# fuine/katome

Hardware: AMD Instinct MI355X
Metric: k-mers/s (higher is better)
Workload: dtype u64

## Files before the change

### katome_amd/csrc/lds_count.hip

```cpp
#include <algorithm>

#include "common.h"
#include "lds_order.h"
#include "lds_plan.h"
#include "slot_bits.h"

namespace katome {

#ifdef KATOME_LC_PHASES
__device__ unsigned long long lc_phase_cycles[16];
#define LC_PHASE_BEGIN() unsigned long long lc_t0 = clock64()
#define LC_PHASE(i) do { if (threadIdx.x == 0) { const unsigned long long lc_t = clock64(); atomicAdd(&lc_phase_cycles[i], lc_t - lc_t0); lc_t0 = lc_t; } } while (0)
#else
#define LC_PHASE_BEGIN() do {} while (0)
#define LC_PHASE(i) do {} while (0)
#endif
template <int PER> KD u32 lc_step(u64 h) {
#ifdef KATOME_LC_LINEAR
    return 1u;
#else
    u32 step = (u32)((h >> 33) & 0x1FFu) * 2u + 1u;
    if ((PER & (PER - 1)) != 0 && step % (u32)PER == 0) step += 2;
    return step;
#endif
}

template <int NW, int STRIDE = NW>
__global__ __launch_bounds__(BLOCK) void hash_group_index_kernel(const u64* __restrict__ keys, u64 n, u32 gbits, u64* __restrict__ index) {
    for (u64 g = (u64)blockIdx.x * BLOCK + threadIdx.x; g <= (1ull << gbits); g += (u64)gridDim.x * BLOCK) {
        u64 lo = 0, hi = n;
        while (lo < hi) {
            const u64 mid = lo + ((hi - lo) >> 1);
            Key<NW> a;
#pragma unroll
            for (int q = 0; q < NW; ++q) a.w[q] = keys[mid * STRIDE + q];
            if ((hash_key(a) >> (64 - gbits)) < g) lo = mid + 1; else hi = mid;
        }
        index[g] = lo;
    }
}

template <bool RC, int PER, bool EVEN_K>
__global__ __launch_bounds__(LC_THREADS) void lds_count_kernel(const u64* keys, const u32* wts, const u64* __restrict__ index, u32 gbits,
                                                                u32 R, u32 k, u32 min_weight, u64* out_keys,
                                                                u32* out_w, u64 out_cap, unsigned long long* cursor,
                                                                unsigned long long* distinct, u32* err, u32 probe_limit,
                                                                unsigned long long* owner_cursor, u32 n_owners) {
    constexpr u32 LC_SLOTS = LcTable<PER>::SLOTS;
    extern __shared__ unsigned long long lc_mem[];
    unsigned long long* lkey = lc_mem;
    u32* lcnt = reinterpret_cast<u32*>(lc_mem + LC_SLOTS);
    __shared__ u32 wtot[LC_THREADS / 64];
    __shared__ unsigned long long base_sh;
    const u32 tid = threadIdx.x, lane = tid & 63, wave = tid >> 6;
    u32 my_distinct = 0;
    LC_PHASE_BEGIN();
    const u32 n_groups = 1u << gbits, sub_shift = 64 - gbits - 16;
    for (u32 g = blockIdx.x; g < n_groups; g += gridDim.x) {
        const u64 lo = index[g], hi = index[g + 1];
        if (lo == hi) continue;
        for (u32 r = 0; r < R; ++r) {
            for (u32 i = tid; i < LC_SLOTS; i += LC_THREADS) { lkey[i] = 0ull; lcnt[i] = 0u; }
            __syncthreads();
            LC_PHASE(0);
            constexpr u32 LU = KATOME_LC_LU;
            for (u64 i0 = lo + tid; i0 < hi; i0 += (u64)LC_THREADS * LU) {
                u64 kv[LU]; u32 wv[LU];
#pragma unroll
// ... 147 lines not shown
                const unsigned long long v = slot[tid * LP_PER + j];
                kk[j].w[0] = 0; cc[j] = 0;
                if (v) {
                    ++my_distinct;
                    cc[j] = (u32)v & 0xFFFFu;
                    kk[j].w[0] = unmix64(((u64)g << 48) | (v >> 16));
                    if (cc[j] >= min_weight) keep |= 1u << j;
                }
            }
            const u32 mine = (u32)__popc(keep);
            u32 incl = mine;
#pragma unroll
            for (int o = 1; o < 64; o <<= 1) { u32 t = __shfl_up(incl, o, 64); if (lane >= (u32)o) incl += t; }
            if (lane == 63) wtot[wave] = incl;
            __syncthreads();
            u32 woff = 0, total = 0;
#pragma unroll
            for (u32 w = 0; w < LC_THREADS / 64; ++w) { if (w < wave) woff += wtot[w]; total += wtot[w]; }
            constexpr u32 F = RC ? 2 : 1;
            if (tid == 0) base_sh = total ? atomicAdd(cursor, (unsigned long long)total * F) : 0ull;
            __syncthreads();
            LC_PHASE(10);
            {
                unsigned long long* skey = lc_mem;
                u32* sw = reinterpret_cast<u32*>(lc_mem + LP_STAGE);
                const u32 p0 = woff + (incl - mine);
                for (u32 c0 = 0; c0 < total; c0 += LP_STAGE) {
                    u32 p = p0 - c0;
#pragma unroll
                    for (u32 j = 0; j < LP_PER; ++j) {
                        if (!((keep >> j) & 1u)) continue;
                        if (p < LP_STAGE) { skey[p] = kk[j].w[0]; sw[p] = cc[j]; }
                        ++p;
                    }
                    __syncthreads();
                    const u32 nc = total - c0 < LP_STAGE ? total - c0 : LP_STAGE;
                    const u64 o0 = base_sh + (u64)c0 * F;
                    for (u32 o = tid; o < nc * F; o += LC_THREADS) {
                        const u32 e = RC ? o >> 1 : o;
                        Key<1> x; x.w[0] = skey[e];
                        if (RC && (o & 1u)) x = revcomp(x, k);
                        if (o0 + o < out_cap) { out_keys[o0 + o] = x.w[0]; out_w[o0 + o] = sw[e]; }
                    }
                    __syncthreads();
                }
            }
            LC_PHASE(11);
        }
    }
    my_distinct = wave_sum(my_distinct);
    if (lane == 0 && my_distinct) atomicAdd(distinct, (unsigned long long)my_distinct);
}

constexpr u32 LO_BUCKETS = LDS_ORDER_BUCKETS;
static_assert(LC_THREADS == LDS_ORDER_THREADS, "the read-out orders with lds_order.h");
template <bool RC>
__global__ __launch_bounds__(LC_THREADS) void lds_count_ordered_kernel(const u64* keys, const u32* wts, const u64* __restrict__ index, u32 k,
                                                                        u32 min_weight, u64* s1_key, u32* s1_w, u32* group_count, u64* s2_key,
                                                                        u32* s2_w, uint8_t* s2_digit, u64 s2_cap, unsigned long long* cursor,
                                                                        unsigned long long* distinct, u32* err, u32 probe_limit) {
    extern __shared__ unsigned long long lc_mem[];
    unsigned long long* slot = lc_mem;
    u32* bucket = reinterpret_cast<u32*>(lc_mem + LP_SLOTS);
    __shared__ u32 wtot[LC_THREADS / 64];
    __shared__ unsigned long long base_sh;
    const u32 tid = threadIdx.x, lane = tid & 63;
    const u32 rem_bits = 2 * k - 16, bshift = rem_bits > 11 ? rem_bits - 11 : 0;
    const u64 REM = (1ull << rem_bits) - 1;
    u32 my_distinct = 0;
    LC_PHASE_BEGIN();
    for (u32 g = blockIdx.x; g < (1u << 16); g += gridDim.x) {
        const u64 lo = index[g], hi = index[g + 1];
        if (lo == hi) continue;
        for (u32 i = tid; i < LP_SLOTS; i += LC_THREADS) slot[i] = 0ull;
        bucket[tid] = 0u;
        __syncthreads();
        LC_PHASE(12);
        constexpr u32 LU = KATOME_LC_LU;
        constexpr u32 NB = LP_SLOTS / 2;
        for (u64 i0 = lo + tid; i0 < hi; i0 += (u64)LC_THREADS * LU) {
            u64 kv[LU]; u32 wv[LU];
#pragma unroll
            for (u32 u = 0; u < LU; ++u) { const u64 i = i0 + (u64)u * LC_THREADS; kv[u] = 0; wv[u] = 0; if (i < hi) { kv[u] = keys[i]; wv[u] = wts[i]; } }
#pragma unroll
            for (u32 u = 0; u < LU; ++u) {
                const u64 i = i0 + (u64)u * LC_THREADS;
                if (i >= hi) continue;
                const u64 h = mix64(kv[u]);
                const u32 w = wv[u];
                if (w == 0u || w > 0xFFFFu) { *err = 5; continue; }
                const unsigned long long rem = kv[u] & REM, mine = (rem << 16) | w;
                u32 b0 = (u32)(((h & 0x3FFFFFFFull) * NB) >> 30);
                const u32 step = lc_step<LP_PER>(h);
                u32 probes = 0;
                for (; probes < probe_limit; ++probes) {
                    u32 b1 = b0 + step; if (b1 >= NB) b1 -= NB;
                    const ulonglong2 x = *reinterpret_cast<const ulonglong2*>(slot + 2 * b0), y = *reinterpret_cast<const ulonglong2*>(slot + 2 * b1);
                    const unsigned long long c[4] = {x.x, x.y, y.x, y.y};
                    u32 at = ~0u; bool have = false;
#pragma unroll
                    for (int j = 3; j >= 0; --j) if ((c[j] >> 16) == rem && c[j] != 0ull) { at = (j < 2 ? 2 * b0 : 2 * b1 - 2) + j; have = true; }
                    if (!have) {
#pragma unroll
                        for (int j = 3; j >= 0; --j) if (c[j] == 0ull) at = (j < 2 ? 2 * b0 : 2 * b1 - 2) + j;
                        if (at == ~0u) { b0 = b1 + step; if (b0 >= NB) b0 -= NB; continue; }
                        const unsigned long long cur = atomicCAS(&slot[at], 0ull, mine);
                        if (cur == 0ull) break;
                        if ((cur >> 16) != rem) continue;
                    }
                    const unsigned long long old = atomicAdd(&slot[at], (unsigned long long)w);
                    if ((old & 0xFFFFull) + w > 0xFFFFull) *err = 5;
                    break;
                }
                if (probes == probe_limit) *err = 3;
            }
        }
        __syncthreads();
        LC_PHASE(13);
        unsigned long long v[LP_PER]; u32 keep = 0;
#pragma unroll
        for (u32 j = 0; j < LP_PER; ++j) {
            v[j] = slot[tid * LP_PER + j];
            if (v[j]) { ++my_distinct; if (((u32)v[j] & 0xFFFFu) >= min_weight) keep |= 1u << j; }
        }
        const u32 total = lds_order_entries<LP_PER>(v, keep, slot, bucket, wtot, bshift, [&](u32 t) {
            if (tid == 0) { group_count[g] = t; base_sh = t ? atomicAdd(cursor, (unsigned long long)t) : 0ull; }
        });
        LC_PHASE(14);
        for (u32 i = tid; i < total; i += LC_THREADS) {
            const unsigned long long e = slot[i];
            Key<1> x; x.w[0] = ((u64)g << rem_bits) | (e >> 16);
            const u32 c = (u32)e & 0xFFFFu;
            if (lo + i < hi) { s1_key[lo + i] = x.w[0]; s1_w[lo + i] = c; }
            if (RC && base_sh + i < s2_cap) {
                const u64 r = revcomp(x, k).w[0];
                s2_key[base_sh + i] = r; s2_w[base_sh + i] = c; s2_digit[base_sh + i] = (uint8_t)(r >> rem_bits);
            }
        }
        __syncthreads();
        LC_PHASE(15);
    }
    my_distinct = wave_sum(my_distinct);
    if (lane == 0 && my_distinct) atomicAdd(distinct, (unsigned long long)my_distinct);
}

template <bool REP>
__global__ __launch_bounds__(BLOCK) void orient_records_kernel(u64* keys, u64 n, u32 k) {
    for (u64 i = (u64)blockIdx.x * BLOCK + threadIdx.x; i < n; i += (u64)gridDim.x * BLOCK) {
        Key<1> x; x.w[0] = keys[i];
        keys[i] = (REP ? rep_orientation(x, k) : canonical(x, k)).w[0];
    }
}

__global__ __launch_bounds__(BLOCK) void core_group_index_kernel(const u64* __restrict__ keys, u64 n, u32 gbits, u32 core_shift, u32 core_bases,
                                                                 u64* __restrict__ index) {
    for (u64 g = (u64)blockIdx.x * BLOCK + threadIdx.x; g <= (1ull << gbits); g += (u64)gridDim.x * BLOCK) {
        u64 lo = 0, hi = n;
        while (lo < hi) {
            const u64 mid = lo + ((hi - lo) >> 1);
            Key<1> a; a.w[0] = keys[mid];
            if ((core_hash(a, core_shift, core_bases) >> (64 - gbits)) < g) lo = mid + 1; else hi = mid;
        }
        index[g] = lo;
    }
}
__global__ void owner_bases_kernel(const u64* __restrict__ index, u32 gbits, u32 n_owners, unsigned long long* owner_cursor, u64* bases) {
    const u32 p = threadIdx.x;
    if (p > n_owners) return;
    const u64 g0 = (((u64)p << gbits) + n_owners - 1) / n_owners;
    const u64 at = index[g0 < (1ull << gbits) ? g0 : (1ull << gbits)];
    bases[p] = at;
    if (p < n_owners) owner_cursor[p] = at;
}

template <bool RC, int PER, int NW, bool EVEN_K>
__global__ __launch_bounds__(LC_THREADS) void lds_count_wide_kernel(const u64* keys, const u32* wts, const u64* __restrict__ index, u32 gbits,
                                                                     u32 R, u32 k, u32 min_weight, u64* out_keys, u32* out_w, u64 out_cap,
                                                                     unsigned long long* cursor, unsigned long long* distinct, u32* err, u32 probe_limit,
                                                                     unsigned long long* , u32 ) {
    constexpr u32 LC_SLOTS = LcTable<PER>::SLOTS;
    constexpr unsigned long long REP_MASK = (1ull << 20) - 1;
    extern __shared__ unsigned long long lc_mem[];
// ... 605 lines not shown
    const uint64_t out_cap = ((rc && !list) ? 2 : 1) * n + 2;
    KCHECK(edge_key.alloc(out_cap * 8 * (list ? stride : nwk), stream));
    KCHECK(seq_weight.alloc(out_cap * (list ? 4 : 16), stream));
    LcResult r;
    auto count = [&](u32 rounds, u32 probe_limit) -> int {
        auto launch = [&](auto kernel) {
            return lc_launch(aux, kernel, (size_t)LcsTable::SLOTS * 28, n, r, ko, wo, index.as<u64>(), gbits, rounds, k, seq_per_read, edge_key.as<u64>(),
                             seq_weight.as<u64>(), out_cap, aux.cursor(), aux.distinct(), aux.err(), probe_limit);
        };
        return with_bool(rc, [&](auto rcv) { return with_bool(list, [&](auto lv) {
            constexpr bool RC = decltype(rcv)::value, LIST = decltype(lv)::value;
            return nwk == 1 ? launch(lds_count_seen_kernel<RC, 1, LIST>) : launch(lds_count_seen_kernel<RC, 2, LIST>);
        }); });
    };
    KCHECK(count_optimistic("first-seen order", lc_rounds_try(avg, lc_optimism(), LcsTable::FILL), R, LcsTable::SLOTS, r, count));
    if (r.code == 4 || r.code == 6) return KATOME_E_UNSUPPORTED;
    if (r.code) { set_error("counting in LDS (first-seen order): a sub-round did not fit its table (code %u)", (unsigned)r.code); return KATOME_E_DEVICE; }
    *n_edges = r.n_out; *n_distinct = r.n_distinct;
    return KATOME_OK;
}

int table_orient_records(uint64_t* d_keys, uint64_t n, uint32_t k, bool rep, hipStream_t stream) {
    if (!n) return KATOME_OK;
    KernelScope ks(K_RECORDS, stream, n);
    if (rep) hipLaunchKernelGGL(orient_records_kernel<true>, dim3(grid_for(n, BLOCK, 256u * 32u)), dim3(BLOCK), 0, stream, d_keys, n, k);
    else     hipLaunchKernelGGL(orient_records_kernel<false>, dim3(grid_for(n, BLOCK, 256u * 32u)), dim3(BLOCK), 0, stream, d_keys, n, k);
    KCHECK_HIP(hipGetLastError());
    return KATOME_OK;
}

static int ordered_count(DevBuf& keys, DevBuf& weights, uint64_t n, uint32_t k, bool rc, uint32_t min_weight, HalfSort& hs, uint64_t* n_edges,
                         uint64_t* n_distinct, hipStream_t stream, uint32_t* first_counts) {
    if (!n || !weights.p || k < 9 || 2 * k > 62 || (rc && !(k & 1)) || !lp_group_fits(n >> 16)) return KATOME_E_UNSUPPORTED;
    const u64* ko = nullptr; const u32* wo = nullptr;
    {
        DevBuf kb(stream), wb(stream);
        KCHECK(kb.alloc((n + 1) * 8)); KCHECK(wb.alloc((n + 1) * 4));
        KCHECK(dev_key_order(keys.as<u64>(), weights.as<u32>(), n, k, kb.as<u64>(), keys.as<u64>(), wb.as<u32>(), weights.as<u32>(), &ko, &wo, stream, first_counts));
    }
    KCHECK(hs.group_first.alloc(((1ull << 16) + 1) * 8, stream));
    KCHECK(dev_key_group_index(ko, n, 2 * k - 16, hs.group_first.as<u64>(), stream));
    KCHECK(hs.group_count.alloc((1ull << 16) * 4, stream));
    KCHECK_HIP(hipMemsetAsync(hs.group_count.p, 0, (1ull << 16) * 4, stream));
    KCHECK(hs.s1_key.alloc((n + 1) * 8, stream)); KCHECK(hs.s1_w.alloc((n + 1) * 4, stream));
    const u64 s2_cap = rc ? n + 1 : 0;
    if (rc) {
        KCHECK(hs.s2_key.alloc(s2_cap * 8, stream)); KCHECK(hs.s2_w.alloc(s2_cap * 4, stream));
        KCHECK(hs.s2_digit.alloc(dev_digit_stream_bytes(s2_cap, 1), stream));
    }
    LcAux aux(stream);
    KCHECK(aux.buf.alloc(64));
    LcResult r;
    KCHECK(with_bool(rc, [&](auto rcv) {
        return lc_launch(aux, lds_count_ordered_kernel<decltype(rcv)::value>, (size_t)LP_SLOTS * 8 + LO_BUCKETS * 2, n, r, ko, wo, hs.group_first.as<u64>(), k,
                         min_weight, hs.s1_key.as<u64>(), hs.s1_w.as<u32>(), hs.group_count.as<u32>(), hs.s2_key.as<u64>(), hs.s2_w.as<u32>(),
                         hs.s2_digit.as<uint8_t>(), s2_cap, aux.cursor(), aux.distinct(), aux.err(), std::min<u32>(lc_probe_limit(), LP_SLOTS));
    }));
    lc_trace("[lds count] in key order, 8-byte slots, 1 visit(s) per record: code %u\n", (unsigned)r.code);
    if (r.code) {
        lc_trace("[lds count] in key order: %s; counting by hash groups\n", r.code == 5 ? "a count over 16 bits" : "a group filled its table");
        hs.release();
        return KATOME_E_UNSUPPORTED;
    }
    hs.n_s1 = r.n_out; hs.n_s2 = rc ? r.n_out : 0; hs.k = k; hs.taken = true;
    *n_edges = hs.n_s1 + hs.n_s2; *n_distinct = r.n_distinct;
    return KATOME_OK;
}

static bool s2_group_sort_on() { static const bool on = env_flag("KATOME_S2_GROUP_SORT", true); return on; }
static uint64_t s2_group_cap() {
    static const uint64_t cap = [] {
        const char* e = getenv("KATOME_S2_GROUP_CAP");
        const uint64_t c = e ? strtoull(e, nullptr, 10) : UINT64_MAX;
        return std::min<uint64_t>(c, dev_group_merge_cap());
    }();
    return cap;
}

int half_sort_finish(HalfSort& hs, DevBuf& edge_key, DevBuf& edge_weight, hipStream_t stream, DevBuf* head_counts) {
    if (head_counts) head_counts->release();
    if (!hs.taken) { set_error("half sort: no ordered count to finish"); return KATOME_E_ARG; }
    const uint32_t k = hs.k;
    DevBuf b_first(stream), a_off(stream);
    KCHECK(b_first.alloc(((1ull << 16) + 1) * 8)); KCHECK(a_off.alloc(((1ull << 16) + 1) * 8));
    bool grouped = false;
    if (hs.n_s2 && s2_group_sort_on()) {
        {
            DevBuf tk(stream), tw(stream);
            KCHECK(tk.alloc((hs.n_s2 + 1) * 8)); KCHECK(tw.alloc((hs.n_s2 + 1) * 4));
            const u64* ko = nullptr; const u32* wo = nullptr;
            KCHECK(dev_key_order(hs.s2_key.as<u64>(), hs.s2_w.as<u32>(), hs.n_s2, k, tk.as<u64>(), hs.s2_key.as<u64>(), tw.as<u32>(),
                                 hs.s2_w.as<u32>(), &ko, &wo, stream, nullptr, hs.s2_digit.as<uint8_t>()));
        }
        hs.s2_digit.release();
        KCHECK(dev_key_group_index(hs.s2_key.as<u64>(), hs.n_s2, 2 * k - 16, b_first.as<u64>(), stream));
        KCHECK(dev_key_group_max(b_first.as<u64>(), a_off.as<u64>(), stream));
        uint64_t largest = 0;
        KCHECK_HIP(hipMemcpyAsync(&largest, a_off.p, 8, hipMemcpyDeviceToHost, stream));
        KCHECK_HIP(hipStreamSynchronize(stream));
        grouped = largest <= s2_group_cap();
        lc_trace("[half sort] S2: %llu keys, largest group %llu: %s\n", (unsigned long long)hs.n_s2, (unsigned long long)largest,
                 grouped ? "ordered per group in the merge" : "too large for the merge's LDS; sorted in full");
        if (!grouped) KCHECK(dev_sort_bufs(hs.s2_key, &hs.s2_w, hs.n_s2, 1, 2 * k, stream, true));
    } else if (hs.n_s2) {
        KCHECK(dev_sort_bufs(hs.s2_key, &hs.s2_w, hs.n_s2, 1, 2 * k, stream, true));
        KCHECK(dev_key_group_index(hs.s2_key.as<u64>(), hs.n_s2, 2 * k - 16, b_first.as<u64>(), stream));
    } else KCHECK_HIP(hipMemsetAsync(b_first.p, 0, b_first.bytes, stream));
// ... 143 lines not shown
    {
        KernelScope ks(K_GROUP_INDEX, stream, n);
        const dim3 igrid(grid_for((1ull << c.gbits) + 1, BLOCK));
        if (split)   hipLaunchKernelGGL(core_group_index_kernel, igrid, dim3(BLOCK), 0, stream, c.ko, n, c.gbits, split->core_shift, split->core_bases, index.as<u64>());
        else if (nw == 1) hipLaunchKernelGGL(hash_group_index_kernel<1>, igrid, dim3(BLOCK), 0, stream, c.ko, n, c.gbits, index.as<u64>());
        else if (nw == 3) hipLaunchKernelGGL(hash_group_index_kernel<3>, igrid, dim3(BLOCK), 0, stream, c.ko, n, c.gbits, index.as<u64>());
        else         hipLaunchKernelGGL(hash_group_index_kernel<2>, igrid, dim3(BLOCK), 0, stream, c.ko, n, c.gbits, index.as<u64>());
    }
    c.out_cap = (rc ? 2 : 1) * n + 1;
    KCHECK(edge_key.alloc(c.out_cap * 8 * nw, stream));
    KCHECK(edge_weight.alloc(c.out_cap * 4, stream));
    c.out_keys = edge_key.as<u64>(); c.out_w = edge_weight.as<u32>();
    if (split) {
        KCHECK(aux.owners.alloc((2 * KATOME_MAX_RANKS + 2) * 8));
        aux.index = c.index; aux.gbits = c.gbits; aux.n_owners = split->n_parts;
    }
    LcResult r;
    bool done = false;
    if (nw == 2) KCHECK(count_whole_keys<WholeKeys2>(c, r, &done));
    if (nw == 3) KCHECK(count_whole_keys<WholeKeys3>(c, r, &done));
    const u32 R_try = lc_rounds_try(c.avg, lc_optimism(), fill);
    if (!done) KCHECK(count_packed(c, R_try, r, &done));
    if (!done) {
        KCHECK(count_optimistic("packed key", R_try, R, ~0u, r, [&](u32 rounds, u32 probe_limit) { return count_sub_rounds(c, rounds, probe_limit, r); }));
        if (r.code == 4) return KATOME_E_UNSUPPORTED;
        if (r.code) { set_error("counting in LDS: a sub-round did not fit its table (code %u)", (unsigned)r.code); return KATOME_E_DEVICE; }
    }
    *n_edges = r.n_out; *n_distinct = r.n_distinct;
    if (split) {
        uint64_t hb[2 * KATOME_MAX_RANKS + 2];
        KCHECK_HIP(hipMemcpyAsync(hb, aux.owners.p, sizeof hb, hipMemcpyDeviceToHost, stream));
        KCHECK_HIP(hipStreamSynchronize(stream));
        uint64_t total = 0;
        for (uint32_t p = 0; p < split->n_parts; ++p) {
            split->base[p] = hb[KATOME_MAX_RANKS + 1 + p];
            split->count[p] = hb[p] - split->base[p];
            total += split->count[p];
        }
        *n_edges = total;
    }
    return KATOME_OK;
}

}

#ifdef KATOME_LC_PHASES
extern "C" int katome_debug_lc_phases(uint64_t* out16) {
    unsigned long long h[16];
    if (hipMemcpyFromSymbol(h, HIP_SYMBOL(katome::lc_phase_cycles), sizeof h) != hipSuccess) return -1;
    for (int i = 0; i < 16; ++i) out16[i] = h[i];
    memset(h, 0, sizeof h);
    return hipMemcpyToSymbol(HIP_SYMBOL(katome::lc_phase_cycles), h, sizeof h) == hipSuccess ? 0 : -1;
}
#endif
```

### katome_amd/csrc/lds_order.h

```cpp
#pragma once

#include "common.h"

namespace katome {

constexpr u32 LDS_ORDER_THREADS = 1024;
constexpr u32 LDS_ORDER_BUCKETS = 2 * LDS_ORDER_THREADS;

template <u32 PER, class OnTotal>
__device__ __forceinline__ u32 lds_order_entries(const unsigned long long (&v)[PER], u32 keep, unsigned long long* slot, u32* bucket,
                                                 u32* wtot, u32 bshift, OnTotal on_total) {
    static_assert(PER * LDS_ORDER_THREADS < (1u << 16), "a group must fit 16-bit bucket counters");
    const u32 tid = threadIdx.x, lane = tid & 63, wave = tid >> 6;
#pragma unroll
    for (u32 j = 0; j < PER; ++j) {
        if (!((keep >> j) & 1u)) continue;
        const u32 b = (u32)((v[j] >> 16) >> bshift);
        atomicAdd(&bucket[b >> 1], 1u << ((b & 1u) * 16u));
    }
    __syncthreads();
    const u32 pair = bucket[tid], lo_cnt = pair & 0xFFFFu, cnt = lo_cnt + (pair >> 16);
    u32 incl = cnt;
#pragma unroll
    for (int o = 1; o < 64; o <<= 1) { u32 t = __shfl_up(incl, o, 64); if (lane >= (u32)o) incl += t; }
    if (lane == 63) wtot[wave] = incl;
    __syncthreads();
    u32 woff = 0, total = 0;
#pragma unroll
    for (u32 w = 0; w < LDS_ORDER_THREADS / 64; ++w) { if (w < wave) woff += wtot[w]; total += wtot[w]; }
    const u32 start = woff + incl - cnt;
    bucket[tid] = start | ((start + lo_cnt) << 16);
    on_total(total);
    __syncthreads();
#pragma unroll
    for (u32 j = 0; j < PER; ++j) {
        if (!((keep >> j) & 1u)) continue;
        const u32 b = (u32)((v[j] >> 16) >> bshift), sh = (b & 1u) * 16u;
        slot[(atomicAdd(&bucket[b >> 1], 1u << sh) >> sh) & 0xFFFFu] = v[j];
    }
    __syncthreads();
    u32 pos[PER];
#pragma unroll
    for (u32 j = 0; j < PER; ++j) {
        pos[j] = 0;
        if (!((keep >> j) & 1u)) continue;
        const u32 b = (u32)((v[j] >> 16) >> bshift), e = (bucket[b >> 1] >> ((b & 1u) * 16u)) & 0xFFFFu;
        u32 r = b ? (bucket[(b - 1) >> 1] >> (((b - 1) & 1u) * 16u)) & 0xFFFFu : 0u;
        const u32 s0 = r;
#pragma unroll 4
        for (u32 i = s0; i < e; ++i) r += slot[i] < v[j] ? 1u : 0u;
        pos[j] = r;
    }
    __syncthreads();
#pragma unroll
    for (u32 j = 0; j < PER; ++j) if ((keep >> j) & 1u) slot[pos[j]] = v[j];
    __syncthreads();
    return total;
}

}
```

### katome_amd/csrc/radix.hip

```cpp
#include <algorithm>
#include <type_traits>

#include "common.h"
#include "lds_order.h"

namespace katome {

constexpr int RADIX_BITS = 8;
constexpr int RADIX = 1 << RADIX_BITS;
#ifndef KATOME_SORT_ITEMS
#define KATOME_SORT_ITEMS 16
#endif
#ifndef KATOME_SORT_ITEMS_WIDE
#define KATOME_SORT_ITEMS_WIDE 8
#endif
#ifndef KATOME_SORT_ITEMS_3
#define KATOME_SORT_ITEMS_3 5
#endif
#ifndef KATOME_SORT_WAVES
#define KATOME_SORT_WAVES 4
#endif
template <int NW> struct SortTile {
    static constexpr int ITEMS = NW == 1 ? KATOME_SORT_ITEMS : NW == 2 ? KATOME_SORT_ITEMS_WIDE : KATOME_SORT_ITEMS_3;
    static constexpr int KEYS = BLOCK * ITEMS;
// ... 847 lines not shown
        const u64 b0 = b_first[g];
        const u64* bp = b_key + b0; const u32* bwp = b_w + b0;
        const u32 na = a_count[g], nb = (u32)(b_first[g + 1] - b0);
        u64 o = a_off[g] + b0;
        u32 ca = 0, cb = 0, la = 0, lb = 0;
        while (ca < na || cb < nb) {
            const u32 ea = na - ca < MW ? na : ca + MW, eb = nb - cb < MW ? nb : cb + MW;
#pragma unroll 4
            for (u32 i = la + tid; i < ea; i += MT) { ak[i & (MW - 1)] = ap[i]; aw[i & (MW - 1)] = awp[i]; }
#pragma unroll 4
            for (u32 i = lb + tid; i < eb; i += MT) { bk[i & (MW - 1)] = bp[i]; bw[i & (MW - 1)] = bwp[i]; }
            la = ea; lb = eb;
            __syncthreads();
            const u32 va = la - ca, vb = lb - cb, c = va + vb < MW ? va + vb : MW;
            const u32 d0 = tid * MI;
            if (d0 < c) {
                u32 lo = d0 > vb ? d0 - vb : 0, hi = d0 < va ? d0 : va;
                while (lo < hi) {
                    const u32 m = (lo + hi) >> 1;
                    if (ak[(ca + m) & (MW - 1)] < bk[(cb + d0 - m - 1) & (MW - 1)]) lo = m + 1; else hi = m;
                }
                u32 i = lo, j = d0 - lo;
                const u32 d1 = d0 + MI < c ? d0 + MI : c;
                for (u32 d = d0; d < d1; ++d) {
                    const bool take_a = i < va && (j >= vb || ak[(ca + i) & (MW - 1)] < bk[(cb + j) & (MW - 1)]);
                    u64 key; u32 w;
                    if (take_a) { key = ak[(ca + i) & (MW - 1)]; w = aw[(ca + i) & (MW - 1)]; ++i; }
                    else        { key = bk[(cb + j) & (MW - 1)]; w = bw[(cb + j) & (MW - 1)]; ++j; }
                    if (o + d < out_cap) { out_key[o + d] = key; out_w[o + d] = w; }
                }
                if (d1 == c) used_a = i;
            }
            __syncthreads();
            ca += used_a; cb += c - used_a; o += c;
            __syncthreads();
        }
    }
}
int dev_half_merge(const uint64_t* a_key, const uint32_t* a_w, const uint64_t* a_first, const uint32_t* a_count, const uint64_t* a_off,
                   const uint64_t* b_key, const uint32_t* b_w, const uint64_t* b_first, uint64_t* out_key, uint32_t* out_w, uint64_t n_out,
                   hipStream_t stream) {
    KernelScope ks(K_HALF_MERGE, stream, n_out);
    hipLaunchKernelGGL(half_merge_kernel, dim3(2048u), dim3(MT), 0, stream, a_key, a_w, a_first, a_count, a_off, b_key, b_w, b_first, out_key, out_w, n_out);
    KCHECK_HIP(hipGetLastError());
    return KATOME_OK;
}

constexpr u32 GM_THREADS = LDS_ORDER_THREADS, GM_PER = 16, GM_WORDS = GM_THREADS * GM_PER, GM_CAP = GM_WORDS - 16;
constexpr u32 GM_STEP = 2048, GM_RING = 2 * GM_STEP, GM_MI = GM_STEP / GM_THREADS, GM_PF = GM_STEP / GM_THREADS;
constexpr size_t GM_LDS = ((size_t)GM_WORDS + GM_RING) * 8;
constexpr u32 SRC_HEAD_BLOCK = 2048;
constexpr u32 GM_SP_WTOT = 0, GM_SP_USED_A = GM_SP_WTOT + GM_THREADS / 64, GM_SP_LAST_E = (GM_SP_USED_A + 1 + 1) / 2 * 2,
              GM_SP_STEP_HEADS = GM_SP_LAST_E + 2 * 2, GM_SP_END = GM_SP_STEP_HEADS + 2;
static_assert(LDS_ORDER_BUCKETS * 2 <= GM_RING * 8 && GM_SP_END <= 2 * (GM_WORDS - GM_CAP), "aliases in the merge's LDS");
template <bool HEADS>
__global__ __launch_bounds__(GM_THREADS) void group_merge_kernel(const u64* __restrict__ a_key, const u32* __restrict__ a_w, const u64* __restrict__ a_first,
                                                                   const u32* __restrict__ a_count, const u64* __restrict__ a_off, const u64* __restrict__ b_key,
                                                                   const u32* __restrict__ b_w, const u64* __restrict__ b_first, u32 k,
                                                                   u64* __restrict__ out_key, u32* __restrict__ out_w, u64 out_cap,
                                                                   u32* __restrict__ head_counts) {
    extern __shared__ unsigned long long gm_mem[];
    unsigned long long* bs = gm_mem;
    u32* spare = reinterpret_cast<u32*>(gm_mem + GM_CAP);
    u32* wtot = spare + GM_SP_WTOT;
    u32* used_a = spare + GM_SP_USED_A;
    unsigned long long* last_e = reinterpret_cast<unsigned long long*>(spare + GM_SP_LAST_E);
    u32* step_heads = spare + GM_SP_STEP_HEADS;
    static_assert(!HEADS || GM_STEP == SRC_HEAD_BLOCK, "a step's outputs lie in at most two blocks of head_counts");
    if (HEADS && threadIdx.x < 2) step_heads[threadIdx.x] = 0u;
    unsigned long long* ring = gm_mem + GM_WORDS;
    u32* bucket = reinterpret_cast<u32*>(ring);
    const u32 tid = threadIdx.x;
    const u32 rem_bits = 2 * k - 16, bshift = rem_bits > 11 ? rem_bits - 11 : 0;
    const u64 REM = (1ull << rem_bits) - 1;
    for (u32 g = blockIdx.x; g < (1u << 16); g += gridDim.x) {
        const u64 b0 = b_first[g], a0 = a_first[g];
        const u32 na = a_count[g], nb = (u32)(b_first[g + 1] - b0);
        const u64* ap = a_key + a0; const u32* awp = a_w + a0;
        u64 o = a_off[g] + b0;
        unsigned long long v[GM_PER]; u32 keep = 0;
#pragma unroll
        for (u32 j = 0; j < GM_PER; ++j) {
            const u32 i = tid + j * GM_THREADS;
            v[j] = 0;
            if (i < nb) { v[j] = ((b_key[b0 + i] & REM) << 16) | b_w[b0 + i]; keep |= 1u << j; }
        }
        bucket[tid] = 0u;
        __syncthreads();
        lds_order_entries<GM_PER>(v, keep, bs, bucket, wtot, bshift, [](u32) {});
        u64 pk[GM_PF]; u32 pw[GM_PF];
        u32 ca = 0, cb = 0, la = 0, pn = na < GM_STEP ? na : GM_STEP;
        u32 step = 0;
#pragma unroll
        for (u32 r = 0; r < GM_PF; ++r) { const u32 i = tid + r * GM_THREADS; if (i < pn) { pk[r] = ap[i]; pw[r] = awp[i]; } }
        while (ca < na || cb < nb) {
            if (pn && la - ca + pn <= GM_RING) {
#pragma unroll
                for (u32 r = 0; r < GM_PF; ++r) {
                    const u32 i = tid + r * GM_THREADS;
                    if (i < pn) ring[(la + i) & (GM_RING - 1)] = ((pk[r] & REM) << 16) | pw[r];
                }
                la += pn;
                pn = na - la < GM_STEP ? na - la : GM_STEP;
#pragma unroll
                for (u32 r = 0; r < GM_PF; ++r) { const u32 i = tid + r * GM_THREADS; if (i < pn) { pk[r] = ap[la + i]; pw[r] = awp[la + i]; } }
            }
            __syncthreads();
            const u32 va = la - ca, vb = nb - cb, c = va + vb < GM_STEP ? va + vb : GM_STEP;
            const u32 d0 = tid * GM_MI;
            u32 h_lo = 0, h_hi = 0;
            if (d0 < c) {
                u32 lo = d0 > vb ? d0 - vb : 0, hi = d0 < va ? d0 : va;
                while (lo < hi) {
                    const u32 m = (lo + hi) >> 1;
                    if (ring[(ca + m) & (GM_RING - 1)] < bs[cb + d0 - m - 1]) lo = m + 1; else hi = m;
                }
                u32 i = lo, j = d0 - lo;
                const u32 d1 = d0 + GM_MI < c ? d0 + GM_MI : c;
                unsigned long long prev = 0;
                bool first = false;
                if (HEADS) {
                    if (d0 == 0) { first = step == 0; if (!first) prev = last_e[(step - 1) & 1]; }
                    else {
                        const unsigned long long pa = i ? ring[(ca + i - 1) & (GM_RING - 1)] : 0ull, pb = j ? bs[cb + j - 1] : 0ull;
                        prev = pa > pb ? pa : pb;
                    }
                }
                for (u32 d = d0; d < d1; ++d) {
                    unsigned long long e;
                    if (i < va && (j >= vb || ring[(ca + i) & (GM_RING - 1)] < bs[cb + j])) e = ring[(ca + i++) & (GM_RING - 1)];
                    else e = bs[cb + j++];
                    if (o + d < out_cap) {
                        out_key[o + d] = ((u64)g << rem_bits) | (e >> 16); out_w[o + d] = (u32)e & 0xFFFFu;
                        if (HEADS && (first || (e >> 18) != (prev >> 18))) {
                            if ((o + d) / SRC_HEAD_BLOCK != o / SRC_HEAD_BLOCK) h_hi |= 1u << (d - d0); else h_lo |= 1u << (d - d0);
                        }
                    }
                    if (HEADS) { prev = e; first = false; }
                }
                if (d1 == c) { *used_a = i; if (HEADS) last_e[step & 1] = prev; }
            }
            if (HEADS) {
                u32 n_lo = 0, n_hi = 0;
#pragma unroll
                for (u32 r = 0; r < GM_MI; ++r) { n_lo += __popcll(__ballot((h_lo >> r) & 1u)); n_hi += __popcll(__ballot((h_hi >> r) & 1u)); }
                if ((tid & 63) == 0) { if (n_lo) atomicAdd(&step_heads[0], n_lo); if (n_hi) atomicAdd(&step_heads[1], n_hi); }
            }
            __syncthreads();
            const u32 ua = *used_a;
            if (HEADS && tid == 0) {
                const u64 blk = o / SRC_HEAD_BLOCK;
                if (step_heads[0]) { atomicAdd(&head_counts[blk], step_heads[0]); step_heads[0] = 0u; }
                if (step_heads[1]) { atomicAdd(&head_counts[blk + 1], step_heads[1]); step_heads[1] = 0u; }
            }
            ca += ua; cb += c - ua; o += c; ++step;
            __syncthreads();
        }
    }
}
uint32_t dev_group_merge_cap() { return GM_CAP; }
uint64_t dev_source_head_blocks(uint64_t n_edges) { return (n_edges + SRC_HEAD_BLOCK - 1) / SRC_HEAD_BLOCK; }
int dev_group_merge(const uint64_t* a_key, const uint32_t* a_w, const uint64_t* a_first, const uint32_t* a_count, const uint64_t* a_off,
                    const uint64_t* b_key, const uint32_t* b_w, const uint64_t* b_first, uint32_t k, uint64_t* out_key, uint32_t* out_w,
                    uint64_t n_out, hipStream_t stream, uint32_t* head_counts) {
    if (k < 9 || 2 * k > 62) { set_error("group merge: k = %u", k); return KATOME_E_ARG; }
    if (head_counts) KCHECK_HIP(hipMemsetAsync(head_counts, 0, dev_source_head_blocks(n_out) * sizeof(u32), stream));
    const auto kernel = head_counts ? group_merge_kernel<true> : group_merge_kernel<false>;
    KCHECK_HIP(hipFuncSetAttribute((const void*)kernel, hipFuncAttributeMaxDynamicSharedMemorySize, (int)GM_LDS));
    KernelScope ks(K_GROUP_MERGE, stream, n_out);
    hipLaunchKernelGGL(kernel, dim3(256u), dim3(GM_THREADS), GM_LDS, stream, a_key, a_w, a_first, a_count, a_off, b_key, b_w, b_first, k, out_key, out_w, n_out,
                       head_counts);
    KCHECK_HIP(hipGetLastError());
    return KATOME_OK;
}

__global__ __launch_bounds__(BLOCK) void key_group_max_kernel(const u64* __restrict__ index, unsigned long long* __restrict__ out) {
    unsigned long long m = 0;
    for (u32 g = blockIdx.x * BLOCK + threadIdx.x; g < (1u << 16); g += gridDim.x * BLOCK) m = max(m, (unsigned long long)(index[g + 1] - index[g]));
#pragma unroll
    for (int o = 32; o > 0; o >>= 1) m = max(m, (unsigned long long)__shfl_xor(m, o, 64));
    if ((threadIdx.x & 63) == 0 && m) atomicMax(out, m);
}
int dev_key_group_max(const uint64_t* d_index, uint64_t* d_out, hipStream_t stream) {
    KCHECK_HIP(hipMemsetAsync(d_out, 0, 8, stream));
    KernelScope ks(K_GROUP_INDEX, stream, 1ull << 16);
    hipLaunchKernelGGL(key_group_max_kernel, dim3(64u), dim3(BLOCK), 0, stream, d_index, reinterpret_cast<unsigned long long*>(d_out));
    KCHECK_HIP(hipGetLastError());
    return KATOME_OK;
}

size_t dev_digit_stream_bytes(uint64_t n, uint32_t nw) { return digit_stream_bytes(n, (int)nw); }
uint32_t dev_sort_tile_keys(uint32_t nw) { return nw == 1 ? SortTile<1>::KEYS : nw == 2 ? SortTile<2>::KEYS : SortTile<3>::KEYS; }
template <int NW>
static int tagged_order_t(const u64* d_in, const u32* w_in, u64 n, u64* ka, u64* kb, u32* wa, u32* wb, const u64** k_out, const u32** w_out, hipStream_t stream,
                          u32* first_counts = nullptr) {
    PassBuffers pb;
    KCHECK(pb.init(n, NW, stream));
    pb.first = first_counts;
    const u64* kin = d_in; const u32* win = w_in;
    u64* kdst[2] = {ka, kb}; u32* wdst[2] = {wa, wb};
    for (int p = 0; p < 2; ++p) {
        HashTaggedDigit<NW> dg{(u32)(64 - 8 * (2 - p))};
        const bool have = p == 0 && first_counts != nullptr;
        if (p == 0 && unstable_first()) {
            if (w_in) KCHECK((radix_pass<NW, true, HashTaggedDigit<NW>, false>(kin, win, n, dg, kdst[p & 1], wdst[p & 1], pb, stream, have)));
            else      KCHECK((radix_pass<NW, false, HashTaggedDigit<NW>, false>(kin, nullptr, n, dg, kdst[p & 1], nullptr, pb, stream, have)));
        } else
        if (w_in) KCHECK((radix_pass<NW, true>(kin, win, n, dg, kdst[p & 1], wdst[p & 1], pb, stream, have)));
        else      KCHECK((radix_pass<NW, false>(kin, nullptr, n, dg, kdst[p & 1], nullptr, pb, stream, have)));
        kin = kdst[p & 1]; win = w_in ? wdst[p & 1] : nullptr;
// ... 992 lines not shown
                  uint32_t* d_edge_weight, uint64_t* d_edge_seq, hipStream_t stream) {
    if (n == 0) return KATOME_OK;
    dim3 grid(grid_for(n, BLOCK)), block(BLOCK);
    if (key_words_for_k(k) == 1) hipLaunchKernelGGL(bfc_edges_kernel<1>, grid, block, 0, stream, d_fwd, d_w, n, k, rc, d_edge_key, d_edge_weight, d_edge_seq);
    else                         hipLaunchKernelGGL(bfc_edges_kernel<2>, grid, block, 0, stream, d_fwd, d_w, n, k, rc, d_edge_key, d_edge_weight, d_edge_seq);
    KCHECK_HIP(hipGetLastError());
    return KATOME_OK;
}

constexpr u32 LABEL_ITEMS = 4;
template <int NW>
__global__ __launch_bounds__(BLOCK) void labels_kernel(const u64* __restrict__ ek, u64 n, u32 k, uint8_t* __restrict__ out) {
    extern __shared__ u32 lbuf[];
    uint8_t* lb = reinterpret_cast<uint8_t*>(lbuf);
    const u32 stride = label_stride_for_k(k), nb = stride - 1, pad = label_pad_for_k(k);
    constexpr u32 TILE = BLOCK * LABEL_ITEMS;
    const u64 ntiles = (n + TILE - 1) / TILE;
    for (u64 t = blockIdx.x; t < ntiles; t += gridDim.x) {
        const u64 e0 = t * TILE;
        const u32 cnt = (u32)((n - e0) < (u64)TILE ? (n - e0) : (u64)TILE);
        Key<NW> key[LABEL_ITEMS];
#pragma unroll
        for (u32 r = 0; r < LABEL_ITEMS; ++r) { const u32 j = r * BLOCK + threadIdx.x; if (j < cnt) key[r] = load_key<NW>(ek, e0 + j); }
#pragma unroll
        for (u32 r = 0; r < LABEL_ITEMS; ++r) {
            const u32 j = r * BLOCK + threadIdx.x;
            if (j < cnt) {
                uint8_t* p = lb + j * stride;
                p[0] = (uint8_t)pad;
                for (u32 i = 0; i < nb; ++i) p[1 + i] = label_byte(key[r], k, i);
            }
        }
        __syncthreads();
        const u64 byte0 = e0 * stride;
        const u32 nbytes = cnt * stride;
        u32* o32 = reinterpret_cast<u32*>(out + byte0);
        for (u32 i = threadIdx.x; i < nbytes / 4; i += BLOCK) o32[i] = lbuf[i];
        for (u32 i = (nbytes / 4) * 4 + threadIdx.x; i < nbytes; i += BLOCK) out[byte0 + i] = lb[i];
        __syncthreads();
    }
}
int dev_labels(const uint64_t* d_edge_key, uint64_t n, uint32_t k, uint8_t* d_label, hipStream_t stream) {
    if (n == 0) return KATOME_OK;
    const size_t lds = (size_t)BLOCK * LABEL_ITEMS * label_stride_for_k(k) + 16;
    dim3 grid(grid_for(n, BLOCK * LABEL_ITEMS, 256u * 16u)), block(BLOCK);
    if ((uintptr_t)d_label % 4) { set_error("label buffer must be 4-byte aligned"); return KATOME_E_ARG; }
    if (key_words_for_k(k) == 1) hipLaunchKernelGGL(labels_kernel<1>, grid, block, lds, stream, d_edge_key, n, k, d_label);
    else                         hipLaunchKernelGGL(labels_kernel<2>, grid, block, lds, stream, d_edge_key, n, k, d_label);
    KCHECK_HIP(hipGetLastError());
    return KATOME_OK;
}

}
```

Baseline: 162.7 billion.

## Use finer bucket ordering and rank by slot position in LDS read-out

```diff
diff --git a/katome_amd/csrc/lds_count.hip b/katome_amd/csrc/lds_count.hip
--- a/katome_amd/csrc/lds_count.hip
+++ b/katome_amd/csrc/lds_count.hip
@@ -11,9 +11,14 @@
 __device__ unsigned long long lc_phase_cycles[16];
 #define LC_PHASE_BEGIN() unsigned long long lc_t0 = clock64()
 #define LC_PHASE(i) do { if (threadIdx.x == 0) { const unsigned long long lc_t = clock64(); atomicAdd(&lc_phase_cycles[i], lc_t - lc_t0); lc_t0 = lc_t; } } while (0)
+__device__ unsigned long long lo_phase_cycles[8];
+#define LO_PHASE_BEGIN() unsigned long long lo_t0 = clock64()
+#define LO_PHASE(i) do { if (threadIdx.x == 0) { const unsigned long long lo_t = clock64(); atomicAdd(&lo_phase_cycles[i], lo_t - lo_t0); lo_t0 = lo_t; } } while (0)
 #else
 #define LC_PHASE_BEGIN() do {} while (0)
 #define LC_PHASE(i) do {} while (0)
+#define LO_PHASE_BEGIN() do {} while (0)
+#define LO_PHASE(i) do {} while (0)
 #endif
 template <int PER> KD u32 lc_step(u64 h) {
 #ifdef KATOME_LC_LINEAR
@@ -267,8 +272,12 @@
     if (lane == 0 && my_distinct) atomicAdd(distinct, (unsigned long long)my_distinct);
 }
 
-constexpr u32 LO_BUCKETS = LDS_ORDER_BUCKETS;
 static_assert(LC_THREADS == LDS_ORDER_THREADS, "the read-out orders with lds_order.h");
+constexpr u32 LO_COARSE_WORDS = (lds_order_words(LDS_ORDER_COARSE_BITS) + 1) / 2 * 2;
+constexpr u32 LO_FINE_SLOT = (LP_SLOTS - (lds_order_words(LDS_ORDER_FINE_BITS) + 1) / 2) / 2 * 2;
+constexpr u32 LO_FINE_MAX = LO_FINE_SLOT;
+constexpr size_t LO_LDS = (size_t)LP_SLOTS * 8 + LO_COARSE_WORDS * 4;
+static_assert((LP_SLOTS - LO_FINE_SLOT) * 2 >= lds_order_words(LDS_ORDER_FINE_BITS), "the fine buckets fit the table's tail");
 template <bool RC>
 __global__ __launch_bounds__(LC_THREADS) void lds_count_ordered_kernel(const u64* keys, const u32* wts, const u64* __restrict__ index, u32 k,
                                                                         u32 min_weight, u64* s1_key, u32* s1_w, u32* group_count, u64* s2_key,
@@ -277,10 +286,14 @@
     extern __shared__ unsigned long long lc_mem[];
     unsigned long long* slot = lc_mem;
     u32* bucket = reinterpret_cast<u32*>(lc_mem + LP_SLOTS);
+    u32* fine = reinterpret_cast<u32*>(lc_mem + LO_FINE_SLOT);
     __shared__ u32 wtot[LC_THREADS / 64];
     __shared__ unsigned long long base_sh;
+    __shared__ u32 kept_sh;
     const u32 tid = threadIdx.x, lane = tid & 63;
-    const u32 rem_bits = 2 * k - 16, bshift = rem_bits > 11 ? rem_bits - 11 : 0;
+    const u32 rem_bits = 2 * k - 16;
+    const u32 bshift_c = rem_bits > LDS_ORDER_COARSE_BITS ? rem_bits - LDS_ORDER_COARSE_BITS : 0;
+    const u32 bshift_f = rem_bits > LDS_ORDER_FINE_BITS ? rem_bits - LDS_ORDER_FINE_BITS : 0;
     const u64 REM = (1ull << rem_bits) - 1;
     u32 my_distinct = 0;
     LC_PHASE_BEGIN();
@@ -289,6 +302,7 @@
         if (lo == hi) continue;
         for (u32 i = tid; i < LP_SLOTS; i += LC_THREADS) slot[i] = 0ull;
         bucket[tid] = 0u;
+        if (tid == 0) kept_sh = 0u;
         __syncthreads();
         LC_PHASE(12);
         constexpr u32 LU = KATOME_LC_LU;
@@ -332,17 +346,31 @@
         }
         __syncthreads();
         LC_PHASE(13);
+        LO_PHASE_BEGIN();
+        u32 rt = tid;
+        asm volatile("" : "+v"(rt));
         unsigned long long v[LP_PER]; u32 keep = 0;
 #pragma unroll
         for (u32 j = 0; j < LP_PER; ++j) {
-            v[j] = slot[tid * LP_PER + j];
+            v[j] = slot[rt * LP_PER + j];
             if (v[j]) { ++my_distinct; if (((u32)v[j] & 0xFFFFu) >= min_weight) keep |= 1u << j; }
         }
-        const u32 total = lds_order_entries<LP_PER>(v, keep, slot, bucket, wtot, bshift, [&](u32 t) {
+        if ((rt + 1) * LP_PER > LO_FINE_SLOT) {
+#pragma unroll
+            for (u32 j = 0; j < LP_PER; ++j) if (rt * LP_PER + j >= LO_FINE_SLOT) slot[rt * LP_PER + j] = 0ull;
+        }
+        const u32 wave_kept = wave_sum((u32)__popc(keep));
+        if (lane == 0 && wave_kept) atomicAdd(&kept_sh, wave_kept);
+        __syncthreads();
+        LO_PHASE(0);
+        const auto reserve = [&](u32 t) {
             if (tid == 0) { group_count[g] = t; base_sh = t ? atomicAdd(cursor, (unsigned long long)t) : 0ull; }
-        });
+        };
+        const auto stamp = [&](u32 i) { LO_PHASE(1 + i); (void)i; };
+        const u32 total = kept_sh <= LO_FINE_MAX ? lds_order_entries<LP_PER, LDS_ORDER_FINE_BITS>(v, keep, slot, fine, wtot, bshift_f, reserve, stamp)
+                                                 : lds_order_entries<LP_PER, LDS_ORDER_COARSE_BITS>(v, keep, slot, bucket, wtot, bshift_c, reserve, stamp);
         LC_PHASE(14);
-        for (u32 i = tid; i < total; i += LC_THREADS) {
+        for (u32 i = rt; i < total; i += LC_THREADS) {
             const unsigned long long e = slot[i];
             Key<1> x; x.w[0] = ((u64)g << rem_bits) | (e >> 16);
             const u32 c = (u32)e & 0xFFFFu;
@@ -1054,7 +1082,7 @@
     KCHECK(aux.buf.alloc(64));
     LcResult r;
     KCHECK(with_bool(rc, [&](auto rcv) {
-        return lc_launch(aux, lds_count_ordered_kernel<decltype(rcv)::value>, (size_t)LP_SLOTS * 8 + LO_BUCKETS * 2, n, r, ko, wo, hs.group_first.as<u64>(), k,
+        return lc_launch(aux, lds_count_ordered_kernel<decltype(rcv)::value>, LO_LDS, n, r, ko, wo, hs.group_first.as<u64>(), k,
                          min_weight, hs.s1_key.as<u64>(), hs.s1_w.as<u32>(), hs.group_count.as<u32>(), hs.s2_key.as<u64>(), hs.s2_w.as<u32>(),
                          hs.s2_digit.as<uint8_t>(), s2_cap, aux.cursor(), aux.distinct(), aux.err(), std::min<u32>(lc_probe_limit(), LP_SLOTS));
     }));
@@ -1304,4 +1332,11 @@
     memset(h, 0, sizeof h);
     return hipMemcpyToSymbol(HIP_SYMBOL(katome::lc_phase_cycles), h, sizeof h) == hipSuccess ? 0 : -1;
 }
+extern "C" int katome_debug_lo_phases(uint64_t* out8) {
+    unsigned long long h[8];
+    if (hipMemcpyFromSymbol(h, HIP_SYMBOL(katome::lo_phase_cycles), sizeof h) != hipSuccess) return -1;
+    for (int i = 0; i < 8; ++i) out8[i] = h[i];
+    memset(h, 0, sizeof h);
+    return hipMemcpyToSymbol(HIP_SYMBOL(katome::lo_phase_cycles), h, sizeof h) == hipSuccess ? 0 : -1;
+}
 #endif
diff --git a/katome_amd/csrc/lds_order.h b/katome_amd/csrc/lds_order.h
--- a/katome_amd/csrc/lds_order.h
+++ b/katome_amd/csrc/lds_order.h
@@ -5,21 +5,36 @@
 namespace katome {
 
 constexpr u32 LDS_ORDER_THREADS = 1024;
-constexpr u32 LDS_ORDER_BUCKETS = 2 * LDS_ORDER_THREADS;
+constexpr u32 LDS_ORDER_COARSE_BITS = 11, LDS_ORDER_FINE_BITS = 13;
+constexpr u32 lds_order_words(u32 bucket_bits) { return (1u << bucket_bits) / 2 + 1; }
+constexpr u32 LDS_ORDER_RANK_UNROLL = 4;
 
-template <u32 PER, class OnTotal>
+template <u32 PER, u32 BB, class OnTotal, class Stamp>
 __device__ __forceinline__ u32 lds_order_entries(const unsigned long long (&v)[PER], u32 keep, unsigned long long* slot, u32* bucket,
-                                                 u32* wtot, u32 bshift, OnTotal on_total) {
+                                                 u32* wtot, u32 bshift, OnTotal on_total, Stamp stamp) {
     static_assert(PER * LDS_ORDER_THREADS < (1u << 16), "a group must fit 16-bit bucket counters");
-    const u32 tid = threadIdx.x, lane = tid & 63, wave = tid >> 6;
+    constexpr u32 NBW = (1u << BB) / 2, WPT = NBW / LDS_ORDER_THREADS;
+    static_assert(WPT == 1 || WPT == 4, "one word or one 16-byte read per thread in the scan");
+    u32 tid = threadIdx.x;
+    asm volatile("" : "+v"(tid));
+    const u32 lane = tid & 63, wave = tid >> 6;
+    u32 arr[(PER + 1) / 2];
+#pragma unroll
+    for (u32 j = 0; j < (PER + 1) / 2; ++j) arr[j] = 0;
 #pragma unroll
     for (u32 j = 0; j < PER; ++j) {
         if (!((keep >> j) & 1u)) continue;
-        const u32 b = (u32)((v[j] >> 16) >> bshift);
-        atomicAdd(&bucket[b >> 1], 1u << ((b & 1u) * 16u));
+        const u32 b = (u32)((v[j] >> 16) >> bshift), sh = (b & 1u) * 16u;
+        arr[j >> 1] |= ((atomicAdd(&bucket[b >> 1], 1u << sh) >> sh) & 0xFFFFu) << ((j & 1u) * 16u);
     }
     __syncthreads();
-    const u32 pair = bucket[tid], lo_cnt = pair & 0xFFFFu, cnt = lo_cnt + (pair >> 16);
+    stamp(0);
+    u32 cw[WPT];
+    if (WPT == 4) { const uint4 q = reinterpret_cast<const uint4*>(bucket)[tid]; cw[0] = q.x; cw[1 % WPT] = q.y; cw[2 % WPT] = q.z; cw[3 % WPT] = q.w; }
+    else cw[0] = bucket[tid];
+    u32 cnt = 0;
+#pragma unroll
+    for (u32 q = 0; q < WPT; ++q) cnt += (cw[q] & 0xFFFFu) + (cw[q] >> 16);
     u32 incl = cnt;
 #pragma unroll
     for (int o = 1; o < 64; o <<= 1) { u32 t = __shfl_up(incl, o, 64); if (lane >= (u32)o) incl += t; }
@@ -28,33 +43,51 @@
     u32 woff = 0, total = 0;
 #pragma unroll
     for (u32 w = 0; w < LDS_ORDER_THREADS / 64; ++w) { if (w < wave) woff += wtot[w]; total += wtot[w]; }
-    const u32 start = woff + incl - cnt;
-    bucket[tid] = start | ((start + lo_cnt) << 16);
+    u32 start = woff + incl - cnt;
+#pragma unroll
+    for (u32 q = 0; q < WPT; ++q) {
+        const u32 lo_cnt = cw[q] & 0xFFFFu, hi_cnt = cw[q] >> 16;
+        cw[q] = start | ((start + lo_cnt) << 16);
+        start += lo_cnt + hi_cnt;
+    }
+    if (WPT == 4) reinterpret_cast<uint4*>(bucket)[tid] = make_uint4(cw[0], cw[1 % WPT], cw[2 % WPT], cw[3 % WPT]);
+    else bucket[tid] = cw[0];
+    if (tid == 0) bucket[NBW] = total | (total << 16);
     on_total(total);
     __syncthreads();
+    stamp(1);
 #pragma unroll
     for (u32 j = 0; j < PER; ++j) {
         if (!((keep >> j) & 1u)) continue;
-        const u32 b = (u32)((v[j] >> 16) >> bshift), sh = (b & 1u) * 16u;
-        slot[(atomicAdd(&bucket[b >> 1], 1u << sh) >> sh) & 0xFFFFu] = v[j];
+        const u32 b = (u32)((v[j] >> 16) >> bshift);
+        slot[((bucket[b >> 1] >> ((b & 1u) * 16u)) & 0xFFFFu) + ((arr[j >> 1] >> ((j & 1u) * 16u)) & 0xFFFFu)] = v[j];
     }
     __syncthreads();
-    u32 pos[PER];
+    stamp(2);
+    unsigned long long e[PER];
 #pragma unroll
-    for (u32 j = 0; j < PER; ++j) {
-        pos[j] = 0;
-        if (!((keep >> j) & 1u)) continue;
-        const u32 b = (u32)((v[j] >> 16) >> bshift), e = (bucket[b >> 1] >> ((b & 1u) * 16u)) & 0xFFFFu;
-        u32 r = b ? (bucket[(b - 1) >> 1] >> (((b - 1) & 1u) * 16u)) & 0xFFFFu : 0u;
-        const u32 s0 = r;
-#pragma unroll 4
-        for (u32 i = s0; i < e; ++i) r += slot[i] < v[j] ? 1u : 0u;
-        pos[j] = r;
+    for (u32 j = 0; j < (PER + 1) / 2; ++j) arr[j] = 0;
+#pragma unroll
+    for (u32 t = 0; t < PER; ++t) {
+        const u32 i = tid + t * LDS_ORDER_THREADS;
+        e[t] = 0;
+        if (i >= total) continue;
+        e[t] = slot[i];
+        const u32 b = (u32)((e[t] >> 16) >> bshift);
+        const unsigned long long two = (unsigned long long)bucket[b >> 1] | ((unsigned long long)bucket[(b >> 1) + 1] << 32);
+        const u32 s = (u32)(two >> ((b & 1u) * 16u)) & 0xFFFFu, en = (u32)(two >> ((b & 1u) * 16u + 16u)) & 0xFFFFu;
+        u32 r = s;
+#pragma unroll
+        for (u32 u = 0; u < LDS_ORDER_RANK_UNROLL; ++u) r += slot[s + u < en ? s + u : i] < e[t] ? 1u : 0u;
+        for (u32 q = s + LDS_ORDER_RANK_UNROLL; q < en; ++q) r += slot[q] < e[t] ? 1u : 0u;
+        arr[t >> 1] |= r << ((t & 1u) * 16u);
     }
     __syncthreads();
+    stamp(3);
 #pragma unroll
-    for (u32 j = 0; j < PER; ++j) if ((keep >> j) & 1u) slot[pos[j]] = v[j];
+    for (u32 t = 0; t < PER; ++t) if (tid + t * LDS_ORDER_THREADS < total) slot[(arr[t >> 1] >> ((t & 1u) * 16u)) & 0xFFFFu] = e[t];
     __syncthreads();
+    stamp(4);
     return total;
 }
 
diff --git a/katome_amd/csrc/radix.hip b/katome_amd/csrc/radix.hip
--- a/katome_amd/csrc/radix.hip
+++ b/katome_amd/csrc/radix.hip
@@ -923,7 +923,15 @@
 constexpr u32 SRC_HEAD_BLOCK = 2048;
 constexpr u32 GM_SP_WTOT = 0, GM_SP_USED_A = GM_SP_WTOT + GM_THREADS / 64, GM_SP_LAST_E = (GM_SP_USED_A + 1 + 1) / 2 * 2,
               GM_SP_STEP_HEADS = GM_SP_LAST_E + 2 * 2, GM_SP_END = GM_SP_STEP_HEADS + 2;
-static_assert(LDS_ORDER_BUCKETS * 2 <= GM_RING * 8 && GM_SP_END <= 2 * (GM_WORDS - GM_CAP), "aliases in the merge's LDS");
+static_assert(lds_order_words(LDS_ORDER_FINE_BITS) * 4 <= GM_RING * 8 && GM_SP_END <= 2 * (GM_WORDS - GM_CAP), "aliases in the merge's LDS");
+#ifdef KATOME_LC_PHASES
+__device__ unsigned long long gm_phase_cycles[8];
+#define GM_PHASE_BEGIN() unsigned long long gm_t0 = clock64()
+#define GM_PHASE(i) do { if (threadIdx.x == 0) { const unsigned long long gm_t = clock64(); atomicAdd(&gm_phase_cycles[i], gm_t - gm_t0); gm_t0 = gm_t; } } while (0)
+#else
+#define GM_PHASE_BEGIN() do {} while (0)
+#define GM_PHASE(i) do {} while (0)
+#endif
 template <bool HEADS>
 __global__ __launch_bounds__(GM_THREADS) void group_merge_kernel(const u64* __restrict__ a_key, const u32* __restrict__ a_w, const u64* __restrict__ a_first,
                                                                    const u32* __restrict__ a_count, const u64* __restrict__ a_off, const u64* __restrict__ b_key,
@@ -942,8 +950,9 @@
     unsigned long long* ring = gm_mem + GM_WORDS;
     u32* bucket = reinterpret_cast<u32*>(ring);
     const u32 tid = threadIdx.x;
-    const u32 rem_bits = 2 * k - 16, bshift = rem_bits > 11 ? rem_bits - 11 : 0;
+    const u32 rem_bits = 2 * k - 16, bshift = rem_bits > LDS_ORDER_FINE_BITS ? rem_bits - LDS_ORDER_FINE_BITS : 0;
     const u64 REM = (1ull << rem_bits) - 1;
+    GM_PHASE_BEGIN();
     for (u32 g = blockIdx.x; g < (1u << 16); g += gridDim.x) {
         const u64 b0 = b_first[g], a0 = a_first[g];
         const u32 na = a_count[g], nb = (u32)(b_first[g + 1] - b0);
@@ -956,9 +965,10 @@
             v[j] = 0;
             if (i < nb) { v[j] = ((b_key[b0 + i] & REM) << 16) | b_w[b0 + i]; keep |= 1u << j; }
         }
-        bucket[tid] = 0u;
+        reinterpret_cast<uint4*>(bucket)[tid] = make_uint4(0u, 0u, 0u, 0u);
         __syncthreads();
-        lds_order_entries<GM_PER>(v, keep, bs, bucket, wtot, bshift, [](u32) {});
+        GM_PHASE(0);
+        lds_order_entries<GM_PER, LDS_ORDER_FINE_BITS>(v, keep, bs, bucket, wtot, bshift, [](u32) {}, [&](u32 i) { GM_PHASE(1 + i); (void)i; });
         u64 pk[GM_PF]; u32 pw[GM_PF];
         u32 ca = 0, cb = 0, la = 0, pn = na < GM_STEP ? na : GM_STEP;
         u32 step = 0;
@@ -1027,6 +1037,7 @@
             ca += ua; cb += c - ua; o += c; ++step;
             __syncthreads();
         }
+        GM_PHASE(6);
     }
 }
 uint32_t dev_group_merge_cap() { return GM_CAP; }
@@ -2125,3 +2136,13 @@
 }
 
 }
+
+#ifdef KATOME_LC_PHASES
+extern "C" int katome_debug_gm_phases(uint64_t* out8) {
+    unsigned long long h[8];
+    if (hipMemcpyFromSymbol(h, HIP_SYMBOL(katome::gm_phase_cycles), sizeof h) != hipSuccess) return -1;
+    for (int i = 0; i < 8; ++i) out8[i] = h[i];
+    memset(h, 0, sizeof h);
+    return hipMemcpyToSymbol(HIP_SYMBOL(katome::gm_phase_cycles), h, sizeof h) == hipSuccess ? 0 : -1;
+}
+#endif
```

After: 171.1 billion (median of 6 runs). 5.2% higher.
